# lisaweijler/SE3Conv3D

Measured on AMD Instinct MI355X. Metric: Mpoints/sec fwd+bwd PNEConvLayerRotEquiv (N=64k,k=32,F=2), higher is better.
Workload: dtype bf16x3 (fp32 split into bf16 hi+lo, 3 MFMA products, fp32 accumulate); 1 GPU; headline: 4-level PNEConvLayerRotEquiv stack, N=65536, k=32, F=2, C=64; conv-only fwd+bwd (dX,dA,dbeta,dW), one scene per GPU; n_points=65536, clouds_per_gpu=1, k=32, frames=2, num_basis=32, point_order=random, launch=hipGraph replay of the captured step, cpu_threads_per_rank=8

## Files before the change

### se3conv3d_amd/csrc/api.hip

```cpp
#include <cstdarg>
#include <cstdio>
#include <cstdlib>
#include <cstring>
#include <map>
#include <mutex>
#include <string>
#include <utility>
#include <vector>

#include "common.h"
#include "../../include/se3conv_forms.h"

namespace se3 {

namespace {
struct FormSink { std::string lines, tag; int n_cu; };
thread_local FormSink* t_forms = nullptr;
}
bool forms_only() { return t_forms != nullptr; }
int forms_cu_count() { return t_forms ? t_forms->n_cu : 0; }
const Switches& switches() {
  static const Switches sw = [] {
    Switches v{};
    v.no_t24 = getenv("SE3_NO_T24") != nullptr;
// ... 295 lines not shown
    const size_t plane = (size_t)s->c_out * align_up((size_t)s->c_in * kb, 32) * 2;
    p.bt_hi = take(plane);
    p.bt_lo = take(plane);
    p.split = take(gemm_nn_bf16_split_bytes((int64_t)s->n_out * s->f_out, s->c_out, s->c_in * (int)kb));
  } else {
    p.split = take(gemm_nn_split_bytes((int64_t)s->n_out * s->f_out, s->c_out, s->c_in * (int)kb));
  }
  p.geom_in = take((size_t)s->n_in * s->f_in * 64);
  p.geom_out = take((size_t)s->n_out * s->f_out * 64);
  p.total = off;
  return p;
}

enum class FeatGrad { none, u, edge_major };
enum class WeightGrad { none, t_saved, t_recomputed, u };

struct BwdPlan {
  bool fast;
  bool feat_branch;
  FeatGrad feat;
  WeightGrad dw;
  bool grad_t;
  bool strip_t;
  int fmt_t, fmt_u;
  struct { int64_t m; int ka, n, splits; } tn;
  int n_param_partials;
  size_t axes_ext, wt, w2, bt_hi, bt_lo, featpk, gpk, split, geom_in, geom_out, big, bx_hi, bx_lo, u, split_x, dx_rows, t,
      param_partials, tn_partials, total;
};
bool plan_edge_major(const se3conv_shape* s, bool want_params) {
  const int mode = switches().dx_path;
  if (mode == 0 || s->precision == SE3_PRECISION_FP32) return false;
  if (s->n_in == 0 || s->n_out == 0) return false;
  if (!edge_dx_bf16_applicable(forward_geom(s), s->c_in)) return false;
  if (s->n_edges * s->f_in * (int64_t)s->c_in >= (1ll << 31)) return false;
  if (mode == 1) return true;
  const double rows_in = (double)s->n_in * s->f_in, rows_out = (double)s->n_out * s->f_out;
  const double u_bytes = rows_in * s->c_out * kBasis * 6.0;
// ... 2 lines not shown
  return 15.0 + d_bytes / 2.2e6 < 45.0 + u_bytes / 6.0e6;
}

BwdPlan plan_bwd(const se3conv_shape* s, bool want_feat, bool want_params, bool have_t) {
  BwdPlan p{};
  const size_t kb = s->num_basis;
  const size_t rows_out = (size_t)s->n_out * s->f_out, rows_in = (size_t)s->n_in * s->f_in;
  const int ck = s->c_in * (int)kb, cok = s->c_out * (int)kb;
  p.fast = s->precision != SE3_PRECISION_FP32;
  p.feat_branch = want_feat && rows_in > 0;
  p.feat = !want_feat ? FeatGrad::none : plan_edge_major(s, want_params) ? FeatGrad::edge_major : FeatGrad::u;
  const bool u_form = p.feat == FeatGrad::u, edge_major = p.feat == FeatGrad::edge_major;
  p.grad_t = want_params || edge_major;
  if (p.fast) {
    p.strip_t = gemm_strip_bf16_applicable((int64_t)rows_out, ck, s->c_out);
    p.fmt_t = t_row_format(s);
    p.fmt_u = row_format(s, transposed_geom(s), s->c_out, 0);
  }
  const bool dw_u = p.fast && u_form && p.feat_branch && want_params && rows_out > 0 && s->c_in % 4 == 0 && s->c_out % 2 == 0 &&
                    (!have_t || (double)rows_in * s->c_out < (double)rows_out * s->c_in);
  p.dw = !want_params ? WeightGrad::none : dw_u ? WeightGrad::u : have_t ? WeightGrad::t_saved : WeightGrad::t_recomputed;
  if (dw_u) p.tn = {(int64_t)rows_in, cok, s->c_in, 0};
  else p.tn = {(int64_t)rows_out, ck, s->c_out, 0};
  p.tn.splits = gemm_tn_splits(p.tn.m, p.tn.ka, p.tn.n);
  p.n_param_partials = edge_param_grad_blocks((int64_t)rows_out);

  size_t off = 0;
  auto take = [&](size_t bytes) { size_t o = off; off = align_up(off + bytes, 256); return o; };
  const size_t wsz = (size_t)s->c_in * kb * s->c_out * 4;
  const size_t t_bytes = rows_out * s->c_in * kb * 4, u_bytes = rows_in * s->c_out * kb * 4;
// ... 432 lines not shown
    if (p.feat_branch) {
      float* u = (float*)(ws + p.u);
      if (int rc = launch_edge_t("edge_t_transposed", gt, grad_out, s->c_out, rows_out, axes_ext, rho, u, stream)) return rc;
      float* w2 = (float*)(ws + p.w2);
      if (!forms_only())
        hipLaunchKernelGGL(permute_weights_oki_kernel, dim3(grid_for((int64_t)ck * s->c_out)), dim3(256), 0, stream,
                           conv_weights, w2, s->c_in, kb, s->c_out);
      if (int rc = launch_gemm_nn("gemm_gradX", u, w2, grad_feat, rows_in, s->c_in, s->c_out * kb, nu, inv_fin, stream,
                                  (float*)(ws + p.split_x)))
        return rc;
    }
    return check_launch();
  }

  const bool u_form = p.feat_branch && p.feat == FeatGrad::u, edge_major = p.feat == FeatGrad::edge_major;
  uint16_t* bt_hi = (uint16_t*)(ws + p.bt_hi);
  uint16_t* bt_lo = (uint16_t*)(ws + p.bt_lo);
  uint16_t* bx_hi = (uint16_t*)(ws + p.bx_hi);
  uint16_t* bx_lo = (uint16_t*)(ws + p.bx_lo);
  uint32_t* gpk = (uint32_t*)(ws + p.gpk);
  const bool have_featpk = prep && prep->feat_words && prep->feat_words_valid;
  uint32_t* featpk = prep && prep->feat_words ? prep->feat_words : (uint32_t*)(ws + p.featpk);
  uint32_t* bigw = (uint32_t*)big;
  uint32_t* u = (uint32_t*)(ws + p.u);
  const float inv_phi = inv_fin / kGeluOut;
  pb.split(grad_out, gpk, rows_out * s->c_out);
  if (u_form) pb.weights(conv_weights, s->c_in, kb, s->c_out, 2, bx_hi, bx_lo, nullptr, 1.0f, false, p.fmt_u);
  if (want_params && !have_featpk) pb.split(feat, featpk, rows_in * s->c_in);
  if (p.grad_t)
    pb.weights(conv_weights, s->c_in, kb, s->c_out, 1, bt_hi, bt_lo, nu, inv_fin, p.strip_t);
  if (int rc = pb.launch(stream)) return rc;
  ReduceBatch final_sums;

  if (u_form) {
    if (int rc = launch_edge_t_bf16("edge_t_transposed", gt, gpk, s->c_out, rows_out, axes_ext, rho, u, stream, p.fmt_u))
      return rc;
  }
  if (p.grad_t) {
    if (int rc = p.strip_t ? launch_gemm_strip_bf16("gemm_gradT", gpk, bt_hi, bt_lo, bigw, rows_out, ck, s->c_out, stream)
                           : launch_gemm_nn_bf16("gemm_gradT", gpk, bt_hi, bt_lo, bigw, true, rows_out, ck, s->c_out,
                                                 (float*)(ws + p.split), nullptr, 1.0f, stream))
      return rc;
  }
  if (edge_major) {
    float* d_rows = (float*)(ws + p.dx_rows);
    if (int rc = launch_edge_dx_bf16("edge_dx", g, axes_ext, rho, bigw, s->c_in, d_rows, stream)) return rc;
    if (int rc = launch_dx_gather_sum("dx_gather", d_rows, neighbors, ends, t_samples, t_ends, t_edge_ids, s->n_in, s->f_in * s->c_in,
                                      1.0f / kGeluOut, grad_feat, stream))
      return rc;
  }
  if (grad_axes || grad_biases) {
    int n_part = 0;
    if (int rc = launch_edge_param_grad_bf16("edge_param_grad", g, featpk, s->c_in, rows_in, axes_ext, rho, bigw, partials,
                                             p.n_param_partials, &n_part, stream))
      return rc;
    final_sums.params(partials, n_part, grad_axes, grad_biases, 0.5f);
  }
  if (u_form) {
    if (int rc = launch_gemm_nn_bf16("gemm_gradX", u, bx_hi, bx_lo, grad_feat, false, rows_in, s->c_in, s->c_out * kb,
                                     (float*)(ws + p.split_x), nu, inv_phi, stream, p.fmt_u, &final_sums))
      return rc;
  }
  if (grad_weights) {
    if (p.dw == WeightGrad::u) {
      if (int rc = launch_gemm_tn_bf16("gemm_gradW", u, featpk, grad_weights, tn_partials, p.tn.splits, p.tn.m, p.tn.ka, p.tn.n,
                                       nu, inv_phi, stream, p.fmt_u, &final_sums, true))
        return rc;
    } else {
      const uint32_t* t = (const uint32_t*)t_save;
// ... 115 lines not shown
```

### se3conv3d_amd/csrc/common.h

```cpp
#pragma once

#include <hip/hip_runtime.h>
#include <stddef.h>
#include <stdint.h>

#include "../../include/se3conv.h"

namespace se3 {

using f32x16 = __attribute__((__vector_size__(16 * sizeof(float)))) float;
using f32x4 = __attribute__((__vector_size__(4 * sizeof(float)))) float;

constexpr int kWave = 64;
constexpr int kBasis = 32;
constexpr int kDescExt = 10;

__host__ __device__ constexpr int acc_row(int reg, int h) { return (reg & 3) + 8 * (reg >> 2) + 4 * h; }

__device__ __forceinline__ f32x16 mfma32(float a, float b, f32x16 c) {
  return __builtin_amdgcn_mfma_f32_32x32x2f32(a, b, c, 0, 0, 0);
}

using bf16x8 = __attribute__((__vector_size__(8 * sizeof(__bf16)))) __bf16;
using bf16x2 = __attribute__((__vector_size__(2 * sizeof(__bf16)))) __bf16;
// ... 329 lines not shown
struct ReduceBatch {
  ReduceJobs jobs{};
  void sum(const float* partials, void* out, int64_t count, int splits, const float* alpha_num, float alpha_scale, bool packed,
           int perm_n = 0);
  void params(const float* partials, int n_partials, float* grad_axes, float* grad_biases, float scale);
  int launch(hipStream_t stream);
};

int launch_split_pack(const float* src, uint32_t* dst, int64_t n, hipStream_t stream);
bool edge_t_bf16_t24_rows(const EdgeGeom& g, int channels);
bool edge_t_bf16_t16_rows(const EdgeGeom& g, int channels);
int launch_edge_t_bf16(const char* tag, const EdgeGeom& g, const uint32_t* feat, int channels, int64_t feat_rows,
                       const float* axes_ext, const float* rho, uint32_t* t_out, hipStream_t stream,
                       int rowfmt = 0);
int edge_param_grad_bf16_channel_blocks(int channels);
int launch_edge_param_grad_bf16(const char* tag, const EdgeGeom& g, const uint32_t* feat, int channels,
                                int64_t feat_rows, const float* axes_ext, const float* rho, const uint32_t* grad_t,
                                float* partials, int n_partials, int* n_used, hipStream_t stream);
bool edge_dx_bf16_applicable(const EdgeGeom& g, int channels);
int launch_edge_dx_bf16(const char* tag, const EdgeGeom& g, const float* axes_ext, const float* rho, const uint32_t* grad_t,
                        int channels, float* d_rows, hipStream_t stream);
int launch_dx_gather_sum(const char* tag, const float* d_rows, const int32_t* neighbors, const int32_t* ends,
                         const int32_t* t_samples, const int32_t* t_ends, const int32_t* t_edge_ids, int64_t n_src, int width,
                         float scale, float* grad_feat, hipStream_t stream);
int launch_prep_weights(const float* w, int c_in, int kb, int c_out, int mode, uint16_t* bt_hi, uint16_t* bt_lo,
                        hipStream_t stream, const float* scale_num = nullptr, float scale = 1.0f,
                        bool frag_layout = false);
__device__ __forceinline__ float knn_dist2(float dx, float dy, float dz) { return fmaf(dz, dz, fmaf(dy, dy, dx * dx)); }
__device__ __forceinline__ int64_t present_rows(const int32_t* __restrict__ n_valid, int64_t n) {
  return n_valid ? max(min((int64_t)*n_valid, n), (int64_t)0) : n;
}
int launch_knn_bruteforce(const float* pts, const int32_t* batch_ids, int64_t n, const float* qpts, const int32_t* qbatch,
                          int64_t m, int k, int32_t* out, hipStream_t stream, const int32_t* n_valid_src = nullptr,
// ... 53 lines not shown
  int p[8];
  float scale;
};
struct PrepJobs {
  int count;
  PrepJob job[8];
};
struct PrepBatch {
  PrepJobs jobs{};
  int status = SE3_OK;
  void axes(const float* axes, const float* biases, float* ext);
  void geometry(const float* pts, const float* frames, int64_t n, int f, float* records);
  void split(const float* src, uint32_t* dst, int64_t n);
  void weights(const float* w, int c_in, int kb, int c_out, int mode, uint16_t* bt_hi, uint16_t* bt_lo,
               const float* scale_num = nullptr, float scale = 1.0f, bool frag_layout = false,
               int a_rowfmt = 0);
  int launch(hipStream_t stream);
};

int launch_pack_geometry(const float* pts, const float* frames, int64_t n, int f, float* records, hipStream_t stream);
bool gemm_strip_bf16_applicable(int64_t m, int n, int k);
int launch_gemm_strip_bf16(const char* tag, const uint32_t* a, const uint16_t* bt_hi, const uint16_t* bt_lo, uint32_t* c,
                           int64_t m, int n, int k, hipStream_t stream);
int launch_gemm_nn_bf16(const char* tag, const uint32_t* a, const uint16_t* bt_hi, const uint16_t* bt_lo, void* c,
                        bool out_packed, int64_t m, int n, int k, float* split_ws, const float* alpha_num,
                        float alpha_scale, hipStream_t stream, int afmt = 0, ReduceBatch* defer = nullptr);
size_t gemm_nn_bf16_split_bytes(int64_t m, int n, int k);
int launch_gemm_tn_bf16(const char* tag, const uint32_t* a, const uint32_t* b, float* c, float* partials, int splits,
                        int64_t m, int ka, int n, const float* alpha_num, float alpha_scale, hipStream_t stream, int afmt = 0,
                        ReduceBatch* defer = nullptr,
                        bool out_ikn = false);

}
```

### se3conv3d_amd/csrc/edge_bf16.hip

```cpp

#include "common.h"
#include "edge_bf16_body.h"

#ifndef SE3_TIMELINE
#define SE3_TIMELINE 0
#endif
#if SE3_TIMELINE
#define TL(...) __VA_ARGS__
namespace se3 {
constexpr int kTlWords = 64;
__device__ uint32_t* g_tl_buf = nullptr;
__device__ uint32_t g_tl_cap = 0;
__device__ __forceinline__ uint32_t tl_now() {
  unsigned long long t;
  __builtin_amdgcn_sched_barrier(0);
  asm volatile("s_memtime %0\n\ts_waitcnt lgkmcnt(0)" : "=s"(t)::"memory");
  __builtin_amdgcn_sched_barrier(0);
  return (uint32_t)t;
}
template <class T>
__device__ __forceinline__ void tl_pin(const T& x) { asm volatile("" ::"v"(x)); }
__device__ __forceinline__ void tl_mark(uint32_t* rec, int slot) { const uint32_t t = tl_now(); if (slot < kTlWords) rec[slot] = t; }
__device__ __forceinline__ void tl_seg(uint32_t* rec, uint32_t& prev, int slot) { const uint32_t t = tl_now(); rec[slot] += t - prev; prev = t; }
__device__ __forceinline__ void tl_flush(int region, uint32_t idx, const uint32_t* rec, int n_words = kTlWords) {
// ... 558 lines not shown
#pragma unroll
  for (int j = 0; j < kDescExt; ++j) {
    const float v = dacc[j] + __shfl_xor(dacc[j], 32);
    if (h == 0) lds_red[wave][j][kcol] = v;
  }
  __syncthreads();
  for (int i = threadIdx.x; i < kDescExt * kBasis; i += blockDim.x) {
    const int j = i / kBasis, k = i % kBasis;
    partials[(int64_t)blockIdx.x * kDescExt * kBasis + i] =
        lds_red[0][j][k] + lds_red[1][j][k] + lds_red[2][j][k] + lds_red[3][j][k];
  }
}

constexpr int kPgPairWaves = 3;
constexpr int kPgSingleWaves = 3;
template <int CH16, int NFR, bool PAIR = false, bool POW2 = false>
__global__ __launch_bounds__(PAIR ? 128 : (NFR == 2 ? 512 : 256), PAIR ? kPgPairWaves : (NFR == 2 ? 2 : (CH16 == 3 ? 3 : kPgSingleWaves))) void edge_param_grad_bf16_v2_kernel(EdgeGeom g, const uint32_t* __restrict__ feat,
                                                                         int row_ch, int64_t feat_rows,
                                                                         const float* __restrict__ axes_ext,
                                                                         const float* __restrict__ rho_p,
                                                                         const uint32_t* __restrict__ grad_t,
                                                                         float* __restrict__ partials, int64_t n_items,
                                                                         int fnb_shift, int64_t item_lo = 0, int pipe = 0) {
  static_assert(!PAIR || NFR == 2, "the pair form shares the two frames of a point");
  constexpr int NW = PAIR ? 2 : (NFR == 2 ? 8 : 4);
  constexpr int NIMG = PAIR ? 1 : NW;
  constexpr int CSTEP = PAIR ? 64 : 32;
  const int c_off = 64 * (int)blockIdx.y;
  const int row_bytes = row_ch * 4;
  __shared__ __attribute__((aligned(16))) uint32_t lds_w[NFR][2][64][4];
  __shared__ __attribute__((aligned(16))) uint16_t lds_desc[NW][NFR][2][32][12];
// ... 16 lines not shown
  const int groups = g.f_ctr / NFR;
  int v_lo = 0, v_hi = 0;
  if (pipe) {
    const int64_t item_f = min((int64_t)blockIdx.x + (int64_t)lane * item_stride, n_items - 1);
    const uint32_t ctr = (uint32_t)(item_lo + (n_items - 1 - item_f)) / (uint32_t)groups;
    v_hi = g.ends[ctr];
    v_lo = g.ends[max((int)ctr - 1, 0)];
    if (ctr == 0) v_lo = 0;
  }
  int64_t item_f = PAIR ? (int64_t)blockIdx.x : (int64_t)blockIdx.x * NW + wave;
  int64_t item = 0;
  int start = 0, n_total = 0, ctr_row = 0, local_j = 0;
  float yc[3], rc[9];
  constexpr int NBUILD = PAIR ? 1 : NFR;
  uint32_t gw[NBUILD][CH16][8];
  int nb_a = 0, nb_b = 0;
  const int c_first = PAIR ? 32 * wave : 0;
  auto nbr_of = [&](int c0) {
    const int fe = min(c0 + kcol, n_total - 1);
    const int e = start + (POW2 || fnb_shift >= 0 ? fe >> fnb_shift : fe / g.f_nb);
    return g.nbr[(int64_t)e * g.nbr_stride + g.nbr_offset];
  };
  auto row_of = [&](int nb, int c0) {
    const int fe = min(c0 + kcol, n_total - 1);
    return (POW2 ? nb << fnb_shift : nb * g.f_nb) + (POW2 || fnb_shift >= 0 ? fe & ((1 << fnb_shift) - 1) : fe % g.f_nb);
  };
  auto find_item = [&]() {
    for (; item_f < n_items; item_f += item_stride, ++local_j) {
      item = item_lo + (n_items - 1 - item_f);
      const int64_t ctr = (uint32_t)item / (uint32_t)groups;
// ... 14 lines not shown
  auto issue_item_loads = [&]() {
    load_geom_record(ctrg_rs, ctr_row, yc, rc);
    nb_a = nbr_of(c_first);
    nb_b = nbr_of(c_first + CSTEP);
  };
  auto issue_image_loads = [&]() {
#pragma unroll
    for (int ab = 0; ab < NBUILD; ++ab) {
      const int a = PAIR ? wave : ab;
      const uint32_t* gt_row = grad_t + ((item * NFR + a) * (int64_t)row_ch + c_off) * kBasis;
      const int row_left = min(row_ch - c_off, 16 * CH16);
      const uint64_t gt_addr = reinterpret_cast<uint64_t>(gt_row);
      const uint64_t gt_base = ((uint64_t)(uint32_t)__builtin_amdgcn_readfirstlane((uint32_t)(gt_addr >> 32)) << 32) |
                               (uint64_t)(uint32_t)__builtin_amdgcn_readfirstlane((uint32_t)gt_addr);
      const __amdgpu_buffer_rsrc_t gt_rs = buffer_of(reinterpret_cast<const void*>(gt_base), (int64_t)row_left * kBasis * 4);
#pragma unroll
      for (int st = 0; st < CH16; ++st)
#pragma unroll
        for (int j = 0; j < 8; ++j)
          gw[ab][st][j] = __builtin_amdgcn_raw_buffer_load_b32(gt_rs, (8 * h * kBasis + kcol) * 4, (16 * st + j) * kBasis * 4, 0);
    }
  };
  int prio_step = wave_slot_id();
  bool have = find_item();
  TL(tl_seg(tl_rec, tl_prev, 1);)
  if (have) issue_item_loads();
  TL(tl_seg(tl_rec, tl_prev, 3);)
  while (have) {
    issue_image_loads();
    TL(tl_pin(nb_a); tl_seg(tl_rec, tl_prev, 4);)
    int q_a = row_of(nb_a, c_first);
    float xn_nx[3], rn_nx[9];
    load_geom_record(nbg_rs, q_a, xn_nx, rn_nx);
    TL(tl_pin(gw[NBUILD - 1][CH16 - 1][7]); tl_seg(tl_rec, tl_prev, 5);)
#pragma unroll
    for (int ab = 0; ab < NBUILD; ++ab)
#pragma unroll
      for (int st = 0; st < CH16; ++st) {
        const int a = PAIR ? wave : ab;
        u32x4 f_hi, f_lo;
        frags_from_words(gw[ab][st], f_hi, f_lo);
        *reinterpret_cast<u32x4*>(&lds_gt[img][a][st][0][lane][0]) = f_hi;
        *reinterpret_cast<u32x4*>(&lds_gt[img][a][st][1][lane][0]) = f_lo;
      }
    TL(tl_seg(tl_rec, tl_prev, 6);)
    if (PAIR) __syncthreads();
    TL(tl_seg(tl_rec, tl_prev, 7);)

    for (int c0 = c_first; c0 < n_total; c0 += CSTEP) {
      rotate_priority(prio_step++);
      const int cnt = min(32, n_total - c0);
      const int qoff = c0 + kcol < n_total ? q_a * row_bytes + c_off * 4 : kOobOffset;
      float d[9];
      const int q_b = row_of(nb_b, c0 + CSTEP);
      nb_b = nbr_of(c0 + 2 * CSTEP);

// ... 174 lines not shown
  return channels >= 64 && !switches().no_pair && !(channels == 64 && g.f_ctr % 2 == 1);
}

bool edge_t_bf16_t24_rows(const EdgeGeom& g, int channels) {
  if (channels % 2 != 0) return false;
  if (edge_t_bf16_uses_pair(g, channels)) return true;
  return channels <= 32 || channels == 64;
}

bool edge_t_bf16_t16_rows(const EdgeGeom& g, int channels) {
  return channels % 64 == 0 && edge_t_bf16_uses_pair(g, channels);
}

static int device_cu_count() {
  if (forms_only()) return forms_cu_count();
  static int n_cu = 0;
  if (n_cu == 0) {
    int dev = 0;
    hipDeviceProp_t prop;
    if (hipGetDevice(&dev) != hipSuccess || hipGetDeviceProperties(&prop, dev) != hipSuccess) return -1;
    n_cu = prop.multiProcessorCount > 0 ? prop.multiProcessorCount : 256;
  }
  return n_cu;
}

struct EdgeTBf16Form {
  enum Kind { stream_pair, pair, stream1, single } kind;
  int ct, nf;
  int vw, fc;
  bool full, p2, t24;
  int tr;
  int shift, rowfmt;
  int64_t items, wgs;
};
static EdgeTBf16Form edge_t_bf16_form(const EdgeGeom& g, int channels, int rowfmt, int n_cu) {
  EdgeTBf16Form f{};
  const int64_t rows = g.n_ctr * g.f_ctr;
  f.rowfmt = rowfmt, f.shift = frame_shift(g.f_nb), f.tr = g.transposed ? 1 : 0;
// ... 115 lines not shown
      SE3_LAUNCH(4, 1, true, false);
      else SE3_LAUNCH_T(2, true);
      else SE3_LAUNCH_T(1, true);
      else SE3_LAUNCH_T(1, false);
      else return SE3_ERR_UNSUPPORTED;
#undef SE3_LAUNCH_T
#undef SE3_LAUNCH
      break;
    }
  }
  return check_launch();
}

int edge_param_grad_bf16_channel_blocks(int channels) { return channels > 64 && channels % 16 == 0 ? (channels + 63) / 64 : 1; }

struct ParamGradBf16Form {
  enum Kind { pair, wave, generic } kind;
  int ch16, nfr;
  bool p2;
  int shift, pipe, blocks_y;
  int64_t items, wgs;
};
static ParamGradBf16Form edge_param_grad_bf16_form(const EdgeGeom& g, int channels, int n_partials, int n_cu) {
  ParamGradBf16Form f{};
  const int64_t rows = g.n_ctr * g.f_ctr;
  f.shift = frame_shift(g.f_nb), f.p2 = f.shift >= 0, f.blocks_y = 1;
  if (!(channels > 0 && (channels % 16 == 0 || channels < 16))) {
    f.kind = ParamGradBf16Form::generic, f.items = rows;
    f.wgs = n_partials < 512 ? n_partials : 512;
    return f;
  }
  const bool two = g.f_ctr % 2 == 0 && !switches().pg_single;
  f.items = two ? rows / 2 : rows;
  f.blocks_y = edge_param_grad_bf16_channel_blocks(channels);
  if (two && (channels >= 64 || channels == 32)) {
    constexpr int per_cu = 6;
    f.kind = ParamGradBf16Form::pair, f.ch16 = channels == 32 ? 2 : 4, f.nfr = 2;
    f.wgs = (int64_t)n_cu * per_cu;
    if (f.wgs > n_partials) f.wgs = n_partials;
    if (f.wgs > f.items) f.wgs = f.items;
    if (f.wgs < 1) f.wgs = 1;
    f.pipe = (f.items + f.wgs - 1) / f.wgs <= 64 && f.items < (1ll << 31) ? 1 : 0;
    return f;
  }
  f.kind = ParamGradBf16Form::wave;
  f.ch16 = channels >= 64 ? 4 : (channels + 15) / 16;
  f.nfr = two ? 2 : 1;
  f.wgs = n_partials < 512 ? n_partials : 512;
  return f;
}

int launch_edge_param_grad_bf16(const char* tag, const EdgeGeom& g, const uint32_t* feat, int channels,
                                int64_t feat_rows, const float* axes_ext, const float* rho, const uint32_t* grad_t,
                                float* partials, int n_partials, int* n_used, hipStream_t stream) {
  const int64_t rows = g.n_ctr * g.f_ctr;
  if (feat_rows * (int64_t)channels * 4 >= (int64_t)kOobOffset) return SE3_ERR_UNSUPPORTED;
  const int n_cu = device_cu_count();
  const ParamGradBf16Form f = edge_param_grad_bf16_form(g, channels, n_partials, n_cu);
  if (f.kind != ParamGradBf16Form::generic && f.items <= 0) {
    *n_used = 0;
    return SE3_OK;
  }
  if (f.kind == ParamGradBf16Form::pair && n_cu <= 0) return SE3_ERR_LAUNCH;
  *n_used = (int)f.wgs * f.blocks_y;
  if (forms_only()) {
    if (f.kind == ParamGradBf16Form::pair)
      return form_report(tag, "param_grad_pair<ch16=%d,p2=%d>/%s/y%d", f.ch16, f.p2, f.pipe ? "pipe" : "loop", f.blocks_y);
    if (f.kind == ParamGradBf16Form::wave)
      return form_report(tag, "param_grad<ch16=%d,nfr=%d,p2=%d>/y%d", f.ch16, f.nfr, f.p2, f.blocks_y);
    return form_report(tag, "param_grad_generic");
  }
  ProfScope prof(tag, stream);
  const int64_t items = f.items;
  const int shift = f.shift, pipe = f.pipe;
  const dim3 grid((unsigned)f.wgs, (unsigned)f.blocks_y);
  switch (f.kind) {
    case ParamGradBf16Form::pair:
#define SE3_PG_PAIR(CH16, P2)                                                                                                 \
  if (f.ch16 == CH16 && f.p2 == P2)                                                                                             \
    hipLaunchKernelGGL((edge_param_grad_bf16_v2_kernel<CH16, 2, true, P2>), grid, dim3(128), 0, stream, g, feat, channels,      \
                       feat_rows, axes_ext, rho, grad_t, partials, items, shift, 0, pipe)
      SE3_PG_PAIR(2, true);
      else SE3_PG_PAIR(2, false);
      else SE3_PG_PAIR(4, true);
      else SE3_PG_PAIR(4, false);
      else return SE3_ERR_UNSUPPORTED;
#undef SE3_PG_PAIR
      break;
    case ParamGradBf16Form::wave:
#define SE3_PG_L(CH16, NFR, P2, THREADS)                                                                                  \
  if (f.ch16 == CH16 && f.nfr == NFR && f.p2 == P2)                                                                         \
    hipLaunchKernelGGL((edge_param_grad_bf16_v2_kernel<CH16, NFR, false, P2>), grid, dim3(THREADS), 0, stream, g, feat, channels, \
                       feat_rows, axes_ext, rho, grad_t, partials, items, shift, 0)
#define SE3_PG1(CH16)                   \
  SE3_PG_L(CH16, 1, true, 256);         \
  else SE3_PG_L(CH16, 1, false, 256)
#define SE3_PG(CH16)                    \
  SE3_PG_L(CH16, 2, true, 512);         \
  else SE3_PG_L(CH16, 2, false, 512);   \
  else SE3_PG1(CH16)
      SE3_PG(1);
      else SE3_PG1(2);
      else SE3_PG(3);
      else SE3_PG1(4);
      else return SE3_ERR_UNSUPPORTED;
#undef SE3_PG
// ... 13 lines not shown
```

### se3conv3d_amd/csrc/gemm_bf16.hip

```cpp
#include <atomic>

#include "common.h"

namespace se3 {

namespace {

constexpr int kGemmDepth = 4;
constexpr int BM = 128, BN = 64, BK = 32;
constexpr int A_LD = BK + 4;
constexpr int B_LD = BK + 8;

__host__ __device__ inline int64_t gemm_a_row_bytes(int afmt, int k) {
  return afmt == 2 ? t16_row_bytes(k / kBasis) : (int64_t)k * (afmt == 1 ? 3 : 4);
}

__device__ __forceinline__ u32x4 ld4_words(const uint32_t* p, int64_t avail, bool vec) {
  if (avail >= 4 && vec) return *reinterpret_cast<const u32x4*>(p);
  const uint32_t x = avail > 0 ? p[0] : 0u, y = avail > 1 ? p[1] : 0u, z = avail > 2 ? p[2] : 0u,
                 w = avail > 3 ? p[3] : 0u;
  return u32x4{x, y, z, w};
}


// ... 405 lines not shown
    __syncthreads();
    if (more) load_super(t1, st + 5);
    compute(1);
    if (more) {
#pragma unroll
      for (int p = 0; p < 4; ++p) ex[p] = ex_next[p];
      store_half(t0, ex, 0, 0, 0);
    }
    __syncthreads();
  }

  nn_store_acc<OUT_MODE, NB>(acc, c, m, n, m0, n0, wave, rl, h, alpha_num, alpha_scale);
}

constexpr int kStripRot = 17;
template <int KS>
__global__ __launch_bounds__(256, KS <= 4 ? 4 : 2) void gemm_strip_bf16_kernel(const uint32_t* __restrict__ a,
                                                                 const uint16_t* __restrict__ bt_hi,
                                                                 const uint16_t* __restrict__ bt_lo,
                                                                 uint32_t* __restrict__ c, int64_t m, int n, int k) {
  constexpr int KP = KS * 16;
  const int lane = threadIdx.x & 63;
  const int wave = __builtin_amdgcn_readfirstlane((int)(threadIdx.x >> 6));
  const int rl = lane & 31, h = lane >> 5;
  const int64_t row0 = (int64_t)blockIdx.x * 128 + wave * 32;
  if (row0 >= m) return;
  const __amdgpu_buffer_rsrc_t a_rs =
      __builtin_amdgcn_make_buffer_rsrc(const_cast<uint32_t*>(a), (short)0, (int)(uint32_t)(m * k * 4), 0x00020000);
  const __amdgpu_buffer_rsrc_t bh_rs = __builtin_amdgcn_make_buffer_rsrc(
      const_cast<uint16_t*>(bt_hi), (short)0, (int)(uint32_t)((int64_t)n * KP * 2), 0x00020000);
  const __amdgpu_buffer_rsrc_t bl_rs = __builtin_amdgcn_make_buffer_rsrc(
// ... 43 lines not shown
      asm volatile("s_waitcnt vmcnt(" #CNT ")"                                                                    \
                   : "+v"(bh[0]), "+v"(bh[1]), "+v"(bh[KS - 2]), "+v"(bh[KS - 1]), "+v"(bl[0]), "+v"(bl[1]),      \
                     "+v"(bl[KS - 2]), "+v"(bl[KS - 1])::"memory");                                               \
    else                                                                                                          \
      asm volatile("s_waitcnt vmcnt(" #CNT ")"                                                                    \
                   : "+v"(bh[0]), "+v"(bh[1]), "+v"(bh[2]), "+v"(bh[3]), "+v"(bh[KS - 4]), "+v"(bh[KS - 3]),      \
                     "+v"(bh[KS - 2]), "+v"(bh[KS - 1]), "+v"(bl[0]), "+v"(bl[1]), "+v"(bl[2]), "+v"(bl[3]),      \
                     "+v"(bl[KS - 4]), "+v"(bl[KS - 3]), "+v"(bl[KS - 2]), "+v"(bl[KS - 1])::"memory");           \
  } while (0)
#pragma unroll
  for (int ks = 0; ks < KS; ++ks) bh[ks] = bl[ks] = u32x4{0u, 0u, 0u, 0u};
  const int64_t c_bytes = (m - row0) * (int64_t)n * 4;
  const __amdgpu_buffer_rsrc_t c_rs = __builtin_amdgcn_make_buffer_rsrc(
      c + row0 * n, (short)0, (int)(uint32_t)(c_bytes > 0xffffffffll ? 0xffffffffll : c_bytes), 0x00020000);
  const int voff = (4 * h * n + rl) * 4;
  const bool cols_full = n % 32 == 0;
  const int n_tiles_all = (n + 31) / 32;
  const int per = (n_tiles_all + (int)gridDim.y - 1) / (int)gridDim.y;
  const int tile_lo = (int)blockIdx.y * per;
  const int n_tiles = min(per, n_tiles_all - tile_lo);
  if (n_tiles <= 0) return;
  const int n_lo = tile_lo * 32, n_hi = min(n, (tile_lo + n_tiles) * 32);
  int n0 = n_lo + (int)(((blockIdx.x * 4 + wave) * (unsigned)kStripRot) % (unsigned)n_tiles) * 32;
  load_b(n0);
  SE3_WAIT_B(0);
  for (int it = 0; it < n_tiles; ++it) {
    f32x16 acc = zero16();
#pragma unroll
    for (int ks = 0; ks < KS; ++ks) acc = mfma_bf16x3(a_hi[ks], a_lo[ks], bh[ks], bl[ks], acc);
    const int n_next = n0 + 32 < n_hi ? n0 + 32 : n_lo;
    load_b(n_next);
    const int lane_off = (cols_full || n0 + rl < n) ? voff : (int)0x7fffff00;
#pragma unroll
    for (int r = 0; r < 16; r += 2) {
      uint32_t w0, w1;
      split_pack2(acc[r], acc[r + 1], w0, w1);
      __builtin_amdgcn_raw_buffer_store_b32(w0, c_rs, lane_off, (acc_row(r, 0) * n + n0) * 4, 0);
      __builtin_amdgcn_raw_buffer_store_b32(w1, c_rs, lane_off, (acc_row(r + 1, 0) * n + n0) * 4, 0);
    }
    SE3_WAIT_B(16);
    n0 = n_next;
  }
#undef SE3_WAIT_B
}

template <bool OUT_PACKED>
__global__ void reduce_splits_kernel(const float* __restrict__ partials, void* __restrict__ out, int64_t count,
                                     int splits, const float* __restrict__ alpha_num, float alpha_scale) {
  const float alpha = (alpha_num ? *alpha_num : 1.0f) * alpha_scale;
  for (int64_t i = (int64_t)blockIdx.x * blockDim.x + threadIdx.x; i < count; i += (int64_t)gridDim.x * blockDim.x) {
    float s = 0.f;
// ... 291 lines not shown
  return kp <= 128 && kp != 96 && n >= 512 && n % 32 == 0 && n <= (1 << 22) && m >= 128 * 16 &&
         (m + 128) * (int64_t)k * 4 < (1ll << 32) - 64 && (int64_t)(n + 64) * kp * 2 < (1ll << 32) - 64;
}

struct GemmStripForm { int ks; dim3 grid; };
static GemmStripForm gemm_strip_bf16_form(int64_t m, int n, int k) {
  const int64_t row_blocks = (m + 127) / 128;
  int n_split = row_blocks >= 1024 ? 1 : (int)(1024 / row_blocks);
  const int n_tiles = n / 32;
  if (n_split > n_tiles / 4) n_split = n_tiles / 4 > 0 ? n_tiles / 4 : 1;
  const int kp = (k + 31) / 32 * 32;
  return {kp == 32 ? 2 : kp == 64 ? 4 : 8, dim3((unsigned)row_blocks, (unsigned)n_split)};
}

int launch_gemm_strip_bf16(const char* tag, const uint32_t* a, const uint16_t* bt_hi, const uint16_t* bt_lo, uint32_t* c,
                           int64_t m, int n, int k, hipStream_t stream) {
  if (m == 0 || n == 0) return SE3_OK;
  if (!gemm_strip_bf16_applicable(m, n, k)) return SE3_ERR_UNSUPPORTED;
  const GemmStripForm f = gemm_strip_bf16_form(m, n, k);
  if (forms_only()) return form_report(tag, "gemm_strip_bf16<ks=%d>", f.ks);
  ProfScope prof(tag, stream);
  const auto kernel = f.ks == 2 ? gemm_strip_bf16_kernel<2> : f.ks == 4 ? gemm_strip_bf16_kernel<4> : gemm_strip_bf16_kernel<8>;
  hipLaunchKernelGGL(kernel, f.grid, dim3(256), 0, stream, a, bt_hi, bt_lo, c, m, n, k);
  return check_launch();
}

struct GemmNnBf16Form {
  int status;
  int afmt, mode, nb;
  bool fast;
  int kp, per, st_per, splits;
  dim3 grid;
};
static GemmNnBf16Form gemm_nn_bf16_form(int64_t m, int n, int k, bool have_split_ws, bool out_packed, int afmt) {
  GemmNnBf16Form f{};
  const bool a24 = afmt == 1, a16 = afmt == 2;
  f.afmt = afmt;
// ... 184 lines not shown
```

### se3conv3d_amd/csrc/prep.hip

```cpp
#include <cstdio>

#include "common.h"

namespace se3 {

namespace {

enum { kJobAxes = 0, kJobGeometry = 1, kJobSplit = 2, kJobWeights = 3 };

__device__ void job_axes(const PrepJob& j, int block, int) {
  const float* axes = (const float*)j.a;
  const float* biases = (const float*)j.b;
  float* ext = (float*)j.o0;
  const int i = block * blockDim.x + threadIdx.x;
  if (i < SE3_DESC_DIMS * kBasis) ext[i] = axes[i];
  else if (i < kDescExt * kBasis) ext[i] = biases[i - SE3_DESC_DIMS * kBasis];
}

__device__ void job_geometry(const PrepJob& j, int block, int blocks) {
  const float* pts = (const float*)j.a;
  const float* frames = (const float*)j.b;
  float* records = (float*)j.o0;
  const int f = j.p[0];
  for (int64_t row = (int64_t)block * blockDim.x + threadIdx.x; row < j.n; row += (int64_t)blocks * blockDim.x) {
// ... 23 lines not shown

__device__ void job_weights(const PrepJob& j, int block, int blocks) {
  const float* w = (const float*)j.a;
  const float* scale_num = (const float*)j.b;
  uint16_t* bt_hi = (uint16_t*)j.o0;
  uint16_t* bt_lo = (uint16_t*)j.o1;
  const int kb = j.p[1], c_out = j.p[2], mode = j.p[3], n = j.p[4], k = j.p[5], kp = j.p[6], frag = j.p[7];
  const float sc = (scale_num ? *scale_num : 1.0f) * j.scale;
  const int64_t total = (int64_t)n * kp;
  for (int64_t idx = (int64_t)block * blockDim.x + threadIdx.x; idx < total; idx += (int64_t)blocks * blockDim.x) {
    const int nn = (int)(idx / kp), kk = (int)(idx % kp);
    float v = 0.f;
    if (kk < k) {
      const int ks = (frag & 2) ? t24_k_of(kk) : ((frag & 4) ? t16_k_of(kk) : kk);
      if (mode == 0) v = w[(int64_t)ks * c_out + nn];
      else if (mode == 1) v = w[(int64_t)nn * c_out + kk];
      else if (mode == 2) v = w[((int64_t)nn * kb + (ks % kb)) * c_out + ks / kb];
      else v = w[((int64_t)kk * kb + (nn % kb)) * c_out + nn / kb];
    }
    const uint32_t pk = split_pack(v * sc);
    const int64_t o = (frag & 1) ? ((((int64_t)(nn / 32) * (kp / 16) + kk / 16) * 64 + ((kk % 16) / 8) * 32 + nn % 32) * 8 + kk % 8)
                           : idx;
    bt_hi[o] = (uint16_t)(pk >> 16);
    bt_lo[o] = (uint16_t)(pk & 0xffffu);
  }
}

__global__ __launch_bounds__(256) void prep_batch_kernel(PrepJobs jobs) {
  int block = blockIdx.x, ji = 0;
  while (ji + 1 < jobs.count && block >= jobs.job[ji].blocks) block -= jobs.job[ji++].blocks;
  const PrepJob& j = jobs.job[ji];
// ... 22 lines not shown
  if (n * f == 0) return;
  if (n * f * 64 >= 0x7fff0000ll) status = SE3_ERR_UNSUPPORTED;
  PrepJob& j = jobs.job[jobs.count++];
  j = PrepJob{};
  j.type = kJobGeometry, j.blocks = blocks_for(n * f, 2048), j.a = pts, j.b = frames, j.o0 = records, j.n = n * f, j.p[0] = f;
}

void PrepBatch::split(const float* src, uint32_t* dst, int64_t n) {
  if (n == 0) return;
  PrepJob& j = jobs.job[jobs.count++];
  j = PrepJob{};
  j.type = kJobSplit, j.blocks = blocks_for((n + 3) / 4, 4096), j.a = src, j.o0 = dst, j.n = n;
}

void PrepBatch::weights(const float* w, int c_in, int kb, int c_out, int mode, uint16_t* bt_hi, uint16_t* bt_lo,
                        const float* scale_num, float scale, bool frag_layout, int a_rowfmt) {
  int n, k;
  if (mode == 0) n = c_out, k = c_in * kb;
  else if (mode == 1) n = c_in * kb, k = c_out;
  else if (mode == 2) n = c_in, k = c_out * kb;
  else n = c_out * kb, k = c_in;
  const int kp = (k + 31) / 32 * 32;
  PrepJob& j = jobs.job[jobs.count++];
  j = PrepJob{};
  j.type = kJobWeights, j.blocks = blocks_for((int64_t)n * kp, 2048), j.a = w, j.b = scale_num, j.o0 = bt_hi, j.o1 = bt_lo;
  j.p[0] = c_in, j.p[1] = kb, j.p[2] = c_out, j.p[3] = mode, j.p[4] = n, j.p[5] = k, j.p[6] = kp, j.p[7] = (frag_layout ? 1 : 0) | (a_rowfmt == 1 ? 2 : 0) | (a_rowfmt == 2 ? 4 : 0);
  j.scale = scale;
}

namespace {
__global__ __launch_bounds__(256) void reduce_batch_kernel(ReduceJobs jobs) {
  __shared__ float red[256];
  int block = blockIdx.x, ji = 0;
  while (ji + 1 < jobs.count && block >= jobs.job[ji].blocks) block -= jobs.job[ji++].blocks;
  const ReduceJob& j = jobs.job[ji];
  if (j.type == 0) {
    const float alpha = (j.alpha_num ? *j.alpha_num : 1.0f) * j.alpha_scale;
    for (int64_t i = (int64_t)block * blockDim.x + threadIdx.x; i < j.count; i += (int64_t)j.blocks * blockDim.x) {
      float s = 0.f;
#pragma unroll 8
      for (int z = 0; z < j.splits; ++z) s += j.partials[(int64_t)z * j.count + i];
// ... 61 lines not shown
  ProfScope prof("reductions", stream);
  hipLaunchKernelGGL(reduce_batch_kernel, dim3((unsigned)total), dim3(256), 0, stream, jobs);
  jobs.count = 0;
  return check_launch();
}

int PrepBatch::launch(hipStream_t stream) {
  if (status != SE3_OK) return status;
  if (jobs.count == 0) return SE3_OK;
  int total = 0;
  for (int i = 0; i < jobs.count; ++i) total += jobs.job[i].blocks;
  if (forms_only()) {
    char kinds[8 * 8 + 1] = {0};
    int n = 0;
    for (int i = 0; i < jobs.count; ++i)
      if (jobs.job[i].type == kJobWeights) n += snprintf(kinds + n, sizeof(kinds) - n, "/w%df%d", jobs.job[i].p[3], jobs.job[i].p[7]);
    return form_report("prep", "prep_batch%s", kinds);
  }
  ProfScope prof("prep", stream);
  hipLaunchKernelGGL(prep_batch_kernel, dim3((unsigned)total), dim3(256), 0, stream, jobs);
  return check_launch();
}


namespace {
__global__ void fill_words_kernel(uint32_t* __restrict__ dst, uint32_t value, int64_t n) {
  for (int64_t i = (int64_t)blockIdx.x * blockDim.x + threadIdx.x; i < n; i += (int64_t)gridDim.x * blockDim.x) dst[i] = value;
}
}

int launch_fill_words(void* dst, uint32_t value, int64_t n_words, hipStream_t stream) {
// ... 9 lines not shown
```

Before: 28.63 Mpoints/s.

## Emit gradT in MFMA fragment order so param-grad loads fragments directly

When the strip GEMM computes grad_t and the edge param-grad v2 kernel consumes it, the weight columns are permuted in prep and the GEMM epilogue swaps hi/lo halves across lanes with DPP. This writes grad_t already in the per-lane hi/lo fragment layout. The param-grad kernel can then load each fragment with two 128-bit buffer loads instead of eight strided 32-bit loads plus a repack. The cost is extra DPP and perm work in the GEMM epilogue, more template instantiations, and a layout coupling between three kernels. It also makes the cached CU count per device and thread-safe.

```diff
diff --git a/se3conv3d_amd/csrc/api.hip b/se3conv3d_amd/csrc/api.hip
--- a/se3conv3d_amd/csrc/api.hip
+++ b/se3conv3d_amd/csrc/api.hip
@@ -333,6 +333,7 @@
 
 enum class FeatGrad { none, u, edge_major };
 enum class WeightGrad { none, t_saved, t_recomputed, u };
+enum class GtOrder { legacy, fragment };
 
 struct BwdPlan {
   bool fast;
@@ -341,6 +342,7 @@
   WeightGrad dw;
   bool grad_t;
   bool strip_t;
+  GtOrder gt_order;
   int fmt_t, fmt_u;
   struct { int64_t m; int ka, n, splits; } tn;
   int n_param_partials;
@@ -373,6 +375,8 @@
   p.grad_t = want_params || edge_major;
   if (p.fast) {
     p.strip_t = gemm_strip_bf16_applicable((int64_t)rows_out, ck, s->c_out);
+    if (p.grad_t && p.strip_t && !edge_major && s->num_basis == kBasis && s->c_in % 16 == 0 && edge_param_grad_bf16_takes_v2(s->c_in))
+      p.gt_order = GtOrder::fragment;
     p.fmt_t = t_row_format(s);
     p.fmt_u = row_format(s, transposed_geom(s), s->c_out, 0);
   }
@@ -835,6 +839,7 @@
   }
 
   const bool u_form = p.feat_branch && p.feat == FeatGrad::u, edge_major = p.feat == FeatGrad::edge_major;
+  const bool gt_fragment = p.gt_order == GtOrder::fragment;
   uint16_t* bt_hi = (uint16_t*)(ws + p.bt_hi);
   uint16_t* bt_lo = (uint16_t*)(ws + p.bt_lo);
   uint16_t* bx_hi = (uint16_t*)(ws + p.bx_hi);
@@ -849,7 +854,7 @@
   if (u_form) pb.weights(conv_weights, s->c_in, kb, s->c_out, 2, bx_hi, bx_lo, nullptr, 1.0f, false, p.fmt_u);
   if (want_params && !have_featpk) pb.split(feat, featpk, rows_in * s->c_in);
   if (p.grad_t)
-    pb.weights(conv_weights, s->c_in, kb, s->c_out, 1, bt_hi, bt_lo, nu, inv_fin, p.strip_t);
+    pb.weights(conv_weights, s->c_in, kb, s->c_out, 1, bt_hi, bt_lo, nu, inv_fin, p.strip_t, 0, gt_fragment);
   if (int rc = pb.launch(stream)) return rc;
   ReduceBatch final_sums;
 
@@ -858,7 +863,7 @@
       return rc;
   }
   if (p.grad_t) {
-    if (int rc = p.strip_t ? launch_gemm_strip_bf16("gemm_gradT", gpk, bt_hi, bt_lo, bigw, rows_out, ck, s->c_out, stream)
+    if (int rc = p.strip_t ? launch_gemm_strip_bf16("gemm_gradT", gpk, bt_hi, bt_lo, bigw, rows_out, ck, s->c_out, stream, gt_fragment)
                            : launch_gemm_nn_bf16("gemm_gradT", gpk, bt_hi, bt_lo, bigw, true, rows_out, ck, s->c_out,
                                                  (float*)(ws + p.split), nullptr, 1.0f, stream))
       return rc;
@@ -873,7 +878,7 @@
   if (grad_axes || grad_biases) {
     int n_part = 0;
     if (int rc = launch_edge_param_grad_bf16("edge_param_grad", g, featpk, s->c_in, rows_in, axes_ext, rho, bigw, partials,
-                                             p.n_param_partials, &n_part, stream))
+                                             p.n_param_partials, &n_part, stream, gt_fragment))
       return rc;
     final_sums.params(partials, n_part, grad_axes, grad_biases, 0.5f);
   }
diff --git a/se3conv3d_amd/csrc/common.h b/se3conv3d_amd/csrc/common.h
--- a/se3conv3d_amd/csrc/common.h
+++ b/se3conv3d_amd/csrc/common.h
@@ -367,9 +367,11 @@
                        const float* axes_ext, const float* rho, uint32_t* t_out, hipStream_t stream,
                        int rowfmt = 0);
 int edge_param_grad_bf16_channel_blocks(int channels);
+bool edge_param_grad_bf16_takes_v2(int channels);
 int launch_edge_param_grad_bf16(const char* tag, const EdgeGeom& g, const uint32_t* feat, int channels,
                                 int64_t feat_rows, const float* axes_ext, const float* rho, const uint32_t* grad_t,
-                                float* partials, int n_partials, int* n_used, hipStream_t stream);
+                                float* partials, int n_partials, int* n_used, hipStream_t stream,
+                                bool gt_fragment = false);
 bool edge_dx_bf16_applicable(const EdgeGeom& g, int channels);
 int launch_edge_dx_bf16(const char* tag, const EdgeGeom& g, const float* axes_ext, const float* rho, const uint32_t* grad_t,
                         int channels, float* d_rows, hipStream_t stream);
@@ -453,14 +455,16 @@
   void split(const float* src, uint32_t* dst, int64_t n);
   void weights(const float* w, int c_in, int kb, int c_out, int mode, uint16_t* bt_hi, uint16_t* bt_lo,
                const float* scale_num = nullptr, float scale = 1.0f, bool frag_layout = false,
-               int a_rowfmt = 0);
+               int a_rowfmt = 0,
+               bool frag_rows = false);
   int launch(hipStream_t stream);
 };
 
 int launch_pack_geometry(const float* pts, const float* frames, int64_t n, int f, float* records, hipStream_t stream);
 bool gemm_strip_bf16_applicable(int64_t m, int n, int k);
 int launch_gemm_strip_bf16(const char* tag, const uint32_t* a, const uint16_t* bt_hi, const uint16_t* bt_lo, uint32_t* c,
-                           int64_t m, int n, int k, hipStream_t stream);
+                           int64_t m, int n, int k, hipStream_t stream,
+                           bool frag_rows = false);
 int launch_gemm_nn_bf16(const char* tag, const uint32_t* a, const uint16_t* bt_hi, const uint16_t* bt_lo, void* c,
                         bool out_packed, int64_t m, int n, int k, float* split_ws, const float* alpha_num,
                         float alpha_scale, hipStream_t stream, int afmt = 0, ReduceBatch* defer = nullptr);
diff --git a/se3conv3d_amd/csrc/edge_bf16.hip b/se3conv3d_amd/csrc/edge_bf16.hip
--- a/se3conv3d_amd/csrc/edge_bf16.hip
+++ b/se3conv3d_amd/csrc/edge_bf16.hip
@@ -1,3 +1,5 @@
+
+#include <atomic>
 
 #include "common.h"
 #include "edge_bf16_body.h"
@@ -596,7 +598,7 @@
 
 constexpr int kPgPairWaves = 3;
 constexpr int kPgSingleWaves = 3;
-template <int CH16, int NFR, bool PAIR = false, bool POW2 = false>
+template <int CH16, int NFR, bool PAIR = false, bool POW2 = false, bool GTF = false>
 __global__ __launch_bounds__(PAIR ? 128 : (NFR == 2 ? 512 : 256), PAIR ? kPgPairWaves : (NFR == 2 ? 2 : (CH16 == 3 ? 3 : kPgSingleWaves))) void edge_param_grad_bf16_v2_kernel(EdgeGeom g, const uint32_t* __restrict__ feat,
                                                                          int row_ch, int64_t feat_rows,
                                                                          const float* __restrict__ axes_ext,
@@ -643,6 +645,7 @@
   float yc[3], rc[9];
   constexpr int NBUILD = PAIR ? 1 : NFR;
   uint32_t gw[NBUILD][CH16][8];
+  u32x4 gf[NBUILD][CH16][2];
   int nb_a = 0, nb_b = 0;
   const int c_first = PAIR ? 32 * wave : 0;
   auto nbr_of = [&](int c0) {
@@ -687,11 +690,19 @@
       const uint64_t gt_base = ((uint64_t)(uint32_t)__builtin_amdgcn_readfirstlane((uint32_t)(gt_addr >> 32)) << 32) |
                                (uint64_t)(uint32_t)__builtin_amdgcn_readfirstlane((uint32_t)gt_addr);
       const __amdgpu_buffer_rsrc_t gt_rs = buffer_of(reinterpret_cast<const void*>(gt_base), (int64_t)row_left * kBasis * 4);
-#pragma unroll
-      for (int st = 0; st < CH16; ++st)
-#pragma unroll
-        for (int j = 0; j < 8; ++j)
-          gw[ab][st][j] = __builtin_amdgcn_raw_buffer_load_b32(gt_rs, (8 * h * kBasis + kcol) * 4, (16 * st + j) * kBasis * 4, 0);
+      if constexpr (GTF) {
+#pragma unroll
+        for (int st = 0; st < CH16; ++st)
+#pragma unroll
+          for (int hl = 0; hl < 2; ++hl)
+            gf[ab][st][hl] = __builtin_amdgcn_raw_buffer_load_b128(gt_rs, lane * 32, st * 2048 + hl * 16, 0);
+      } else {
+#pragma unroll
+        for (int st = 0; st < CH16; ++st)
+#pragma unroll
+          for (int j = 0; j < 8; ++j)
+            gw[ab][st][j] = __builtin_amdgcn_raw_buffer_load_b32(gt_rs, (8 * h * kBasis + kcol) * 4, (16 * st + j) * kBasis * 4, 0);
+      }
     }
   };
   int prio_step = wave_slot_id();
@@ -705,14 +716,15 @@
     int q_a = row_of(nb_a, c_first);
     float xn_nx[3], rn_nx[9];
     load_geom_record(nbg_rs, q_a, xn_nx, rn_nx);
-    TL(tl_pin(gw[NBUILD - 1][CH16 - 1][7]); tl_seg(tl_rec, tl_prev, 5);)
+    TL(if constexpr (!GTF) tl_pin(gw[NBUILD - 1][CH16 - 1][7]); tl_seg(tl_rec, tl_prev, 5);)
 #pragma unroll
     for (int ab = 0; ab < NBUILD; ++ab)
 #pragma unroll
       for (int st = 0; st < CH16; ++st) {
         const int a = PAIR ? wave : ab;
         u32x4 f_hi, f_lo;
-        frags_from_words(gw[ab][st], f_hi, f_lo);
+        if constexpr (GTF) f_hi = gf[ab][st][0], f_lo = gf[ab][st][1];
+        else frags_from_words(gw[ab][st], f_hi, f_lo);
         *reinterpret_cast<u32x4*>(&lds_gt[img][a][st][0][lane][0]) = f_hi;
         *reinterpret_cast<u32x4*>(&lds_gt[img][a][st][1][lane][0]) = f_lo;
       }
@@ -917,14 +929,19 @@
 
 static int device_cu_count() {
   if (forms_only()) return forms_cu_count();
-  static int n_cu = 0;
-  if (n_cu == 0) {
-    int dev = 0;
-    hipDeviceProp_t prop;
-    if (hipGetDevice(&dev) != hipSuccess || hipGetDeviceProperties(&prop, dev) != hipSuccess) return -1;
-    n_cu = prop.multiProcessorCount > 0 ? prop.multiProcessorCount : 256;
-  }
-  return n_cu;
+  static std::atomic<int> n_cu[64];
+  int dev = 0;
+  if (hipGetDevice(&dev) != hipSuccess) return -1;
+  const bool slot = dev >= 0 && dev < 64;
+  if (slot) {
+    const int known = n_cu[dev].load(std::memory_order_relaxed);
+    if (known > 0) return known;
+  }
+  int count = 0;
+  if (hipDeviceGetAttribute(&count, hipDeviceAttributeMultiprocessorCount, dev) != hipSuccess) return -1;
+  if (count <= 0) count = 256;
+  if (slot) n_cu[dev].store(count, std::memory_order_relaxed);
+  return count;
 }
 
 struct EdgeTBf16Form {
@@ -1070,6 +1087,8 @@
 
 int edge_param_grad_bf16_channel_blocks(int channels) { return channels > 64 && channels % 16 == 0 ? (channels + 63) / 64 : 1; }
 
+bool edge_param_grad_bf16_takes_v2(int channels) { return channels > 0 && (channels % 16 == 0 || channels < 16); }
+
 struct ParamGradBf16Form {
   enum Kind { pair, wave, generic } kind;
   int ch16, nfr;
@@ -1081,7 +1100,7 @@
   ParamGradBf16Form f{};
   const int64_t rows = g.n_ctr * g.f_ctr;
   f.shift = frame_shift(g.f_nb), f.p2 = f.shift >= 0, f.blocks_y = 1;
-  if (!(channels > 0 && (channels % 16 == 0 || channels < 16))) {
+  if (!edge_param_grad_bf16_takes_v2(channels)) {
     f.kind = ParamGradBf16Form::generic, f.items = rows;
     f.wgs = n_partials < 512 ? n_partials : 512;
     return f;
@@ -1108,11 +1127,12 @@
 
 int launch_edge_param_grad_bf16(const char* tag, const EdgeGeom& g, const uint32_t* feat, int channels,
                                 int64_t feat_rows, const float* axes_ext, const float* rho, const uint32_t* grad_t,
-                                float* partials, int n_partials, int* n_used, hipStream_t stream) {
+                                float* partials, int n_partials, int* n_used, hipStream_t stream, bool gt_fragment) {
   const int64_t rows = g.n_ctr * g.f_ctr;
   if (feat_rows * (int64_t)channels * 4 >= (int64_t)kOobOffset) return SE3_ERR_UNSUPPORTED;
   const int n_cu = device_cu_count();
   const ParamGradBf16Form f = edge_param_grad_bf16_form(g, channels, n_partials, n_cu);
+  if (gt_fragment && (f.kind == ParamGradBf16Form::generic || channels % 16 != 0)) return SE3_ERR_UNSUPPORTED;
   if (f.kind != ParamGradBf16Form::generic && f.items <= 0) {
     *n_used = 0;
     return SE3_OK;
@@ -1133,7 +1153,10 @@
   switch (f.kind) {
     case ParamGradBf16Form::pair:
 #define SE3_PG_PAIR(CH16, P2)                                                                                                 \
-  if (f.ch16 == CH16 && f.p2 == P2)                                                                                             \
+  if (f.ch16 == CH16 && f.p2 == P2 && gt_fragment)                                                                              \
+    hipLaunchKernelGGL((edge_param_grad_bf16_v2_kernel<CH16, 2, true, P2, true>), grid, dim3(128), 0, stream, g, feat, channels, \
+                       feat_rows, axes_ext, rho, grad_t, partials, items, shift, 0, pipe);                                      \
+  else if (f.ch16 == CH16 && f.p2 == P2)                                                                                        \
     hipLaunchKernelGGL((edge_param_grad_bf16_v2_kernel<CH16, 2, true, P2>), grid, dim3(128), 0, stream, g, feat, channels,      \
                        feat_rows, axes_ext, rho, grad_t, partials, items, shift, 0, pipe)
       SE3_PG_PAIR(2, true);
@@ -1145,7 +1168,10 @@
       break;
     case ParamGradBf16Form::wave:
 #define SE3_PG_L(CH16, NFR, P2, THREADS)                                                                                  \
-  if (f.ch16 == CH16 && f.nfr == NFR && f.p2 == P2)                                                                         \
+  if (f.ch16 == CH16 && f.nfr == NFR && f.p2 == P2 && gt_fragment)                                                          \
+    hipLaunchKernelGGL((edge_param_grad_bf16_v2_kernel<CH16, NFR, false, P2, true>), grid, dim3(THREADS), 0, stream, g, feat, channels, \
+                       feat_rows, axes_ext, rho, grad_t, partials, items, shift, 0);                                        \
+  else if (f.ch16 == CH16 && f.nfr == NFR && f.p2 == P2)                                                                    \
     hipLaunchKernelGGL((edge_param_grad_bf16_v2_kernel<CH16, NFR, false, P2>), grid, dim3(THREADS), 0, stream, g, feat, channels, \
                        feat_rows, axes_ext, rho, grad_t, partials, items, shift, 0)
 #define SE3_PG1(CH16)                   \
diff --git a/se3conv3d_amd/csrc/gemm_bf16.hip b/se3conv3d_amd/csrc/gemm_bf16.hip
--- a/se3conv3d_amd/csrc/gemm_bf16.hip
+++ b/se3conv3d_amd/csrc/gemm_bf16.hip
@@ -443,7 +443,7 @@
 }
 
 constexpr int kStripRot = 17;
-template <int KS>
+template <int KS, bool FRAG = false>
 __global__ __launch_bounds__(256, KS <= 4 ? 4 : 2) void gemm_strip_bf16_kernel(const uint32_t* __restrict__ a,
                                                                  const uint16_t* __restrict__ bt_hi,
                                                                  const uint16_t* __restrict__ bt_lo,
@@ -517,6 +517,8 @@
   const __amdgpu_buffer_rsrc_t c_rs = __builtin_amdgcn_make_buffer_rsrc(
       c + row0 * n, (short)0, (int)(uint32_t)(c_bytes > 0xffffffffll ? 0xffffffffll : c_bytes), 0x00020000);
   const int voff = (4 * h * n + rl) * 4;
+  const bool lo_lane = (rl & 4) != 0;
+  const uint32_t sel0 = lo_lane ? 0x01000504u : 0x05040100u, sel1 = lo_lane ? 0x03020706u : 0x07060302u;
   const bool cols_full = n % 32 == 0;
   const int n_tiles_all = (n + 31) / 32;
   const int per = (n_tiles_all + (int)gridDim.y - 1) / (int)gridDim.y;
@@ -537,7 +539,17 @@
 #pragma unroll
     for (int r = 0; r < 16; r += 2) {
       uint32_t w0, w1;
-      split_pack2(acc[r], acc[r + 1], w0, w1);
+      if constexpr (FRAG) {
+        uint32_t hi, lo;
+        split2(acc[r], acc[r + 1], hi, lo);
+        const uint32_t send = lo_lane ? hi : lo, keep = lo_lane ? lo : hi;
+        uint32_t recv = (uint32_t)__builtin_amdgcn_update_dpp((int)send, (int)send, 0x104, 0xf, 0x5, false);
+        recv = (uint32_t)__builtin_amdgcn_update_dpp((int)recv, (int)send, 0x114, 0xf, 0xa, false);
+        w0 = __builtin_amdgcn_perm(recv, keep, sel0);
+        w1 = __builtin_amdgcn_perm(recv, keep, sel1);
+      } else {
+        split_pack2(acc[r], acc[r + 1], w0, w1);
+      }
       __builtin_amdgcn_raw_buffer_store_b32(w0, c_rs, lane_off, (acc_row(r, 0) * n + n0) * 4, 0);
       __builtin_amdgcn_raw_buffer_store_b32(w1, c_rs, lane_off, (acc_row(r + 1, 0) * n + n0) * 4, 0);
     }
@@ -859,13 +871,15 @@
 }
 
 int launch_gemm_strip_bf16(const char* tag, const uint32_t* a, const uint16_t* bt_hi, const uint16_t* bt_lo, uint32_t* c,
-                           int64_t m, int n, int k, hipStream_t stream) {
+                           int64_t m, int n, int k, hipStream_t stream, bool frag_rows) {
   if (m == 0 || n == 0) return SE3_OK;
   if (!gemm_strip_bf16_applicable(m, n, k)) return SE3_ERR_UNSUPPORTED;
+  if (frag_rows && n % (16 * kBasis) != 0) return SE3_ERR_UNSUPPORTED;
   const GemmStripForm f = gemm_strip_bf16_form(m, n, k);
   if (forms_only()) return form_report(tag, "gemm_strip_bf16<ks=%d>", f.ks);
   ProfScope prof(tag, stream);
-  const auto kernel = f.ks == 2 ? gemm_strip_bf16_kernel<2> : f.ks == 4 ? gemm_strip_bf16_kernel<4> : gemm_strip_bf16_kernel<8>;
+  const auto kernel = frag_rows ? (f.ks == 2 ? gemm_strip_bf16_kernel<2, true> : f.ks == 4 ? gemm_strip_bf16_kernel<4, true> : gemm_strip_bf16_kernel<8, true>)
+                                : (f.ks == 2 ? gemm_strip_bf16_kernel<2> : f.ks == 4 ? gemm_strip_bf16_kernel<4> : gemm_strip_bf16_kernel<8>);
   hipLaunchKernelGGL(kernel, f.grid, dim3(256), 0, stream, a, bt_hi, bt_lo, c, m, n, k);
   return check_launch();
 }
diff --git a/se3conv3d_amd/csrc/prep.hip b/se3conv3d_amd/csrc/prep.hip
--- a/se3conv3d_amd/csrc/prep.hip
+++ b/se3conv3d_amd/csrc/prep.hip
@@ -61,7 +61,11 @@
     if (kk < k) {
       const int ks = (frag & 2) ? t24_k_of(kk) : ((frag & 4) ? t16_k_of(kk) : kk);
       if (mode == 0) v = w[(int64_t)ks * c_out + nn];
-      else if (mode == 1) v = w[(int64_t)nn * c_out + kk];
+      else if (mode == 1) {
+        const int t = nn >> 5, rl = nn & 31;
+        const int ns = (frag & 8) ? (8 * (t >> 3) + 2 * (rl & 3) + ((rl >> 2) & 1)) * kBasis + 4 * (t & 7) + (rl >> 3) : nn;
+        v = w[(int64_t)ns * c_out + kk];
+      }
       else if (mode == 2) v = w[((int64_t)nn * kb + (ks % kb)) * c_out + ks / kb];
       else v = w[((int64_t)kk * kb + (nn % kb)) * c_out + nn / kb];
     }
@@ -114,7 +118,7 @@
 }
 
 void PrepBatch::weights(const float* w, int c_in, int kb, int c_out, int mode, uint16_t* bt_hi, uint16_t* bt_lo,
-                        const float* scale_num, float scale, bool frag_layout, int a_rowfmt) {
+                        const float* scale_num, float scale, bool frag_layout, int a_rowfmt, bool frag_rows) {
   int n, k;
   if (mode == 0) n = c_out, k = c_in * kb;
   else if (mode == 1) n = c_in * kb, k = c_out;
@@ -124,7 +128,7 @@
   PrepJob& j = jobs.job[jobs.count++];
   j = PrepJob{};
   j.type = kJobWeights, j.blocks = blocks_for((int64_t)n * kp, 2048), j.a = w, j.b = scale_num, j.o0 = bt_hi, j.o1 = bt_lo;
-  j.p[0] = c_in, j.p[1] = kb, j.p[2] = c_out, j.p[3] = mode, j.p[4] = n, j.p[5] = k, j.p[6] = kp, j.p[7] = (frag_layout ? 1 : 0) | (a_rowfmt == 1 ? 2 : 0) | (a_rowfmt == 2 ? 4 : 0);
+  j.p[0] = c_in, j.p[1] = kb, j.p[2] = c_out, j.p[3] = mode, j.p[4] = n, j.p[5] = k, j.p[6] = kp, j.p[7] = (frag_layout ? 1 : 0) | (a_rowfmt == 1 ? 2 : 0) | (a_rowfmt == 2 ? 4 : 0) | (frag_rows ? 8 : 0);
   j.scale = scale;
 }
 
@@ -216,7 +220,7 @@
     char kinds[8 * 8 + 1] = {0};
     int n = 0;
     for (int i = 0; i < jobs.count; ++i)
-      if (jobs.job[i].type == kJobWeights) n += snprintf(kinds + n, sizeof(kinds) - n, "/w%df%d", jobs.job[i].p[3], jobs.job[i].p[7]);
+      if (jobs.job[i].type == kJobWeights) n += snprintf(kinds + n, sizeof(kinds) - n, "/w%df%d", jobs.job[i].p[3], jobs.job[i].p[7] & 7);
     return form_report("prep", "prep_batch%s", kinds);
   }
   ProfScope prof("prep", stream);
```

After: 28.68 Mpoints/s, median of 5. About the same (+0.2%).
